# DocF/multispectral-object-detection

Measured on AMD Instinct MI355X. Metric: image-pairs/sec fwd, yolov5l+CFTx3 640×640 bs64, 1/2/4/8 GPU, higher is better.
Workload: dtype bf16; 1 GPU; cfg3 (yolov5l_fusion_transformerx3_FLIR_aligned) two-stream forward, 640x640, 64 pairs/GPU, BN folded, pre-NMS detections; pairs_per_gpu=64, image_size=640, parallelism=batch-shard x1, hip_graph=True, two_hip_streams=False, forwards_in_flight=3, streams_per_forward_in_flight=1, single_in_flight_streams=2

## Files before the change

include/cft_hip.h:

```cpp
#ifndef CFT_HIP_H
#define CFT_HIP_H

#ifdef __cplusplus
extern "C" {
#endif

#define CFT_ABI_VERSION 17

enum { CFT_BF16 = 0, CFT_F32 = 1, CFT_F16 = 2 };
enum { CFT_ACT_NONE = 0, CFT_ACT_SILU = 1, CFT_ACT_GELU = 2 };
enum {
  CFT_OK = 0,
  CFT_EINVAL = -1,
  CFT_ELAUNCH = -2,
  CFT_ENODEV = -3
};

int cft_abi_version(void);
int cft_device_check(void);
const char* cft_last_error(void);
int cft_clock_probe(void* out4_u64, int spin_us, int* wall_khz, void* stream);

int cft_conv2d(const void* x, const void* w, const float* bias, const void* res, void* y,
               int B, int H, int W, int cin, int ldx, int xoff,
               int n, int kpad, int ksize, int stride,
               int ldy, int yoff, int ldr, int roff,
               int act, int dtype, int out_dtype, int res_dtype, void* stream);

int cft_conv2d_chain(const void* x, const void* w1, const float* bias1, const void* w2, const float* bias2, void* y,
                     int B, int H, int W, int cin, int ldx, int xoff,
                     int n1, int kpad1, int ksize, int stride, int n2,
                     int ldy, int yoff, int act2, int dtype, void* stream);
int cft_conv2d_chain_ok(int B, int H, int W, int cin, int ldx, int n1, int kpad1, int ksize, int stride, int n2, int ldy, int dtype);

int cft_conv2d_chain_res(const void* x, const void* w1, const float* bias1, const void* res, void* y1,
                         const void* w2, const float* bias2, void* y2,
                         int B, int H, int W, int cin, int ldx, int xoff,
                         int n1, int kpad1, int ksize, int stride, int ldr, int roff, int ldy1, int yoff1,
                         int n2, int ldy2, int yoff2, int act2, int dtype, void* stream);

// ... 26 lines not shown
int cft_to_nhwc(const void* in, int in_dtype, long stride_b, long stride_c, long stride_h, long stride_w,
                void* out, int ldo, int ooff, int B, int C, int cpad, int H, int W, int dtype, void* stream);

int cft_letterbox_u8(const unsigned char* src, int src_h, int src_w, long src_row_stride,
                     unsigned char* dst, int dst_h, int dst_w, long dst_stride_y, long dst_stride_x, long dst_stride_c, int flip_channels,
                     int resized_h, int resized_w, int top, int left, int color0, int color1, int color2, void* stream);

enum { CFT_PAIR_COPY = 0, CFT_PAIR_LINEAR = 1, CFT_PAIR_AREA = 2 };
#define CFT_PAIR_DESC_BYTES 64
#define CFT_PAIR_MAX_REDUCTION 4
typedef struct {
  const unsigned char* src_rgb;
  const unsigned char* src_ir;
  long stride_rgb, stride_ir;
  int h0, w0;
  int h, w;
  int top, left;
  int mode, flip;
} cft_pair_desc_t;
int cft_pair_batch_u8(const void* desc_dev, const void* desc_host, int B, unsigned char* dst, int dst_h, int dst_w, int color, void* stream);

int cft_add(const void* a, int lda, int aoff, const void* b, int ldb, int boff,
            void* out, int ldo, int ooff, long M, int C, int dtype, void* stream);

int cft_gpt_tokenize(const void* rgb, int ld_rgb, int off_rgb, const void* ir, int ld_ir, int off_ir,
                     const float* pos_emb, float* tokens, int B, int H, int W, int C,
                     int dtype, void* stream);

int cft_layernorm(const float* x, const float* gamma, const float* beta, void* y,
                  long rows, int C, float eps, int out_dtype, void* stream);
int cft_layernorm_reduce(float* x, const float* parts, int nparts, const float* gamma, const float* beta, void* y,
                         long rows, int C, float eps, int out_dtype, void* stream);

int cft_attention(const void* qkv, void* out, int B, int heads, int dk, int dkp,
                  int dtype, float attn_pdrop, unsigned long long seed, void* stream);

int cft_gpt_upsample_add(const float* tokens, int s, const void* base, int ldb, int boff,
                         void* out, int ldo, int ooff, int B, int H, int W, int C,
                         int dtype, void* stream);

int cft_gpt_upsample_add2(const float* tokens, const void* base0, int ldb0, int boff0, const void* base1, int ldb1, int boff1,
                          void* out0, int ldo0, int ooff0, void* out1, int ldo1, int ooff1, void* sum, int lds, int soff,
                          int B, int H, int W, int C, int dtype, void* stream);

int cft_gpt_tokenize_grid(const void* rgb, int ld_rgb, int off_rgb, const void* ir, int ld_ir, int off_ir,
                          const float* pos_emb, float* tokens, int B, int H, int W, int C, int va, int ha,
                          int dtype, void* stream);

int cft_attention_tokens(const void* qkv, void* out, int B, int T, int heads, int dk, int dkp,
                         int dtype, float attn_pdrop, unsigned long long seed, void* stream);

int cft_gpt_upsample_add_grid(const float* tokens, int s, const void* base, int ldb, int boff,
                              void* out, int ldo, int ooff, int B, int H, int W, int C, int va, int ha,
                              int dtype, void* stream);

int cft_gpt_upsample_add2_grid(const float* tokens, const void* base0, int ldb0, int boff0, const void* base1, int ldb1, int boff1,
                               void* out0, int ldo0, int ooff0, void* out1, int ldo1, int ooff1, void* sum, int lds, int soff,
                               int B, int H, int W, int C, int va, int ha, int dtype, void* stream);

int cft_detect_decode(const float* logits, int ldl, float* raw, float* pred, const float* anchors,
                      int B, int ny, int nx, int na, int no, float stride,
                      long row0, long total_rows, void* stream);

long cft_batchnorm_train_workspace(long M, int C);
int cft_batchnorm_train(const float* x, int ldx, int xoff, long M, int C,
                        const float* gamma, const float* beta, float* running_mean, float* running_var,
// ... 48 lines not shown
```

multispectral-object-detection_amd/_lib.py:

```python
import ctypes
import os
import re
import subprocess

import torch

_HERE = os.path.dirname(os.path.abspath(__file__))
LIB_PATH = os.environ.get("CFT_HIP_LIB") or os.path.join(_HERE, "libcft_hip.so")
CSRC = os.path.join(_HERE, "csrc")
SOURCES = ("runtime.hip", "conv_gemm.hip", "conv_gemm_asm.hip", "focus_conv.hip", "bottleneck.hip", "pointwise.hip", "attention.hip", "attention_tokens.hip", "nms.hip", "train.hip", "metrics.hip", "confusion.hip", "loss.hip", "autoanchor.hip", "dataset.hip")

HEADER = os.path.join(_HERE, "..", "include", "cft_hip.h")
HEADERS = ("cft_common.h", "conv_common.h", "focus_common.h", "bneck_common.h", "metrics_common.h", "resize_common.h", "conv_gemm_asm.inc")

_SCALARS = {"int": ctypes.c_int, "long": ctypes.c_long, "float": ctypes.c_float, "unsigned long long": ctypes.c_ulonglong}
_RETURNS = {"int": ctypes.c_int, "long": ctypes.c_long, "const char*": ctypes.c_char_p}
_TYPE_WORDS = frozenset("void char short int long float double signed unsigned const".split())


def parse_header(text):
    text = re.sub(r"/\*.*?\*/|//[^\n]*", " ", text, flags=re.S)
    consts = {k: int(v) for k, v in re.findall(r"(?:#define\s+|\b)(CFT_\w+)\s*=?\s*(-?\d+)\b", text)}
    text = re.sub(r"^\s*#.*$", "", text, flags=re.M)
    sigs = {}
    for ret, name, args in re.findall(r"([\w\s*]+?)\b(cft_\w+)\s*\(([^()]*)\)\s*;", text):
        ret = re.sub(r"\s*\*", "*", " ".join(ret.split()))
        if ret not in _RETURNS:
            raise ValueError(f"{name}: unknown return type '{ret}'")
        argtypes = []
        for arg in ([] if args.strip() in ("", "void") else args.split(",")):
            *kind, pname = [w for w in arg.split() if w != "const"] or [""]
            if "*" in arg:
                argtypes.append(ctypes.c_void_p)
            elif " ".join(kind) in _SCALARS and pname not in _TYPE_WORDS:
                argtypes.append(_SCALARS[" ".join(kind)])
            else:
                raise ValueError(f"{name}: unknown parameter type in '{' '.join(arg.split())}' (scalars are named int / long / float / unsigned long long)")
        sigs[name] = (_RETURNS[ret], argtypes)
    return sigs, consts


with open(HEADER) as _fh:
    SIGNATURES, _consts = parse_header(_fh.read())
# ... 60 lines not shown
```

multispectral-object-detection_amd/csrc/cft_common.h:

```cpp
#pragma once
#include <hip/hip_runtime.h>
#include <stdint.h>
#include "../../include/cft_hip.h"

typedef __attribute__((ext_vector_type(8))) __bf16 bf16x8_t;
typedef __attribute__((ext_vector_type(4))) float f32x4_t;
typedef _Float16 f16_t;
typedef __attribute__((ext_vector_type(8))) _Float16 f16x8_t;
typedef __attribute__((ext_vector_type(2))) _Float16 f16x2_t;

typedef __attribute__((ext_vector_type(4))) uint32_t gran_t;

__device__ __forceinline__ float bf16_to_f32(uint16_t h) { return __uint_as_float(((uint32_t)h) << 16); }
__device__ __forceinline__ uint16_t f32_to_bf16(float f) {
  uint32_t u = __float_as_uint(f);
  if ((u & 0x7fffffffu) > 0x7f800000u) return (uint16_t)((u >> 16) | 0x40);
  u += 0x7fffu + ((u >> 16) & 1u);
  return (uint16_t)(u >> 16);
}
typedef __attribute__((ext_vector_type(2))) __bf16 bf16x2_t;
typedef __attribute__((ext_vector_type(2))) float f32x2_t;
__device__ __forceinline__ uint32_t pack_bf16x2(float lo, float hi) {
  return __builtin_bit_cast(uint32_t, __builtin_convertvector(f32x2_t{lo, hi}, bf16x2_t));
}
// ... 61 lines not shown
}
template <>
__device__ __forceinline__ f32x4_t mma_granule<f16_t>(const gran_t& a, const gran_t& b, f32x4_t c) {
  return __builtin_amdgcn_mfma_f32_16x16x32_f16(__builtin_bit_cast(f16x8_t, a), __builtin_bit_cast(f16x8_t, b), c, 0, 0, 0);
}
template <>
__device__ __forceinline__ f32x4_t mma_granule<float>(const gran_t& a, const gran_t& b, f32x4_t c) {
#pragma unroll
  for (int j = 0; j < 4; ++j)
    c = __builtin_amdgcn_mfma_f32_16x16x4f32(__uint_as_float(a[j]), __uint_as_float(b[j]), c, 0, 0, 0);
  return c;
}

__device__ __forceinline__ void lds_barrier() {
  asm volatile("s_waitcnt lgkmcnt(0)\n\ts_barrier" ::: "memory");
}

template <int ACT>
__device__ __forceinline__ float apply_act(float v) {
  if constexpr (ACT == CFT_ACT_SILU) return v * __builtin_amdgcn_rcpf(1.0f + __expf(-v));
  if constexpr (ACT == CFT_ACT_GELU) {
    const float z = fabsf(v) * 0.70710678118654752f;
    const float t = __builtin_amdgcn_rcpf(fmaf(0.3275911f, z, 1.0f));
    const float e = __builtin_amdgcn_exp2f(z * (z * -1.4426950408889634f));
    float q = fmaf(1.061405429f, t, -1.453152027f);
    q = fmaf(q, t, 1.421413741f);
    q = fmaf(q, t, -0.284496736f);
    q = fmaf(q, t, 0.254829592f);
    return fmaf(-0.5f * fabsf(v), q * t * e, fmaxf(v, 0.0f));
  }
  return v;
}

__device__ __forceinline__ uint32_t cft_hash32(unsigned long long seed, unsigned long long i) {
  unsigned long long z = seed + (i + 1ull) * 0x9E3779B97F4A7C15ull;
  z = (z ^ (z >> 30)) * 0xBF58476D1CE4E5B9ull;
  z = (z ^ (z >> 27)) * 0x94D049BB133111EBull;
  z = z ^ (z >> 31);
  return (uint32_t)(z >> 32);
}

void cft_set_error(const char* msg);
int cft_check_launch(const char* what);
static inline hipStream_t as_stream(void* s) { return (hipStream_t)s; }

template <auto Kernel>
static inline void cft_allow_lds(int bytes) {
  static bool done[64] = {};
  int dev = 0;
  if (hipGetDevice(&dev) != hipSuccess || dev < 0 || dev >= 64) {
    (void)hipFuncSetAttribute(reinterpret_cast<const void*>(Kernel), hipFuncAttributeMaxDynamicSharedMemorySize, bytes);
    return;
  }
  if (!done[dev]) {
    (void)hipFuncSetAttribute(reinterpret_cast<const void*>(Kernel), hipFuncAttributeMaxDynamicSharedMemorySize, bytes);
    done[dev] = true;
  }
}

static inline bool cft_is_dtype(int d) { return d == CFT_BF16 || d == CFT_F16 || d == CFT_F32; }
static inline int cft_elem_size(int d) { return d == CFT_F32 ? 4 : 2; }
static inline int cft_granule(int d) { return d == CFT_F32 ? 4 : 8; }

#define CFT_DISPATCH_DTYPE(dt_, T, ...)                              \
  do {                                                               \
    if ((dt_) == CFT_BF16) { using T = uint16_t; __VA_ARGS__; }      \
// ... 12 lines not shown
```

multispectral-object-detection_amd/csrc/pointwise.hip:

```cpp
#include "cft_common.h"
#include "resize_common.h"

static inline int grid_for(long work, int block) {
  long g = (work + block - 1) / block;
  const long cap = 256L * 16;
  return (int)(g < 1 ? 1 : (g > cap ? cap : g));
}

template <typename T>
__global__ void __launch_bounds__(256) focus_s2d_kernel(const float* __restrict__ in, unsigned char* __restrict__ out,
                                                        int B, int H, int W) {
  const int Ho = H >> 1, Wo = W >> 1;
  const long total = (long)B * Ho * Wo;
  for (long idx = (long)blockIdx.x * blockDim.x + threadIdx.x; idx < total; idx += (long)gridDim.x * blockDim.x) {
    const int x = (int)(idx % Wo);
    const long t = idx / Wo;
    const int y = (int)(t % Ho);
    const int b = (int)(t / Ho);
    float v[16];
#pragma unroll
    for (int c = 0; c < 3; ++c) {
      const float* base = in + (((long)b * 3 + c) * H + 2 * y) * W + 2 * x;
      const float2 top = *reinterpret_cast<const float2*>(base);
      const float2 bot = *reinterpret_cast<const float2*>(base + W);
// ... 328 lines not shown
        Elem<T>::unpack(*reinterpret_cast<const gran_t*>(src + (((long)b * H + y) * W + x) * ldb + offb + cg * 16L), f);
#pragma unroll
        for (int e = 0; e < GE; ++e) acc[e] += f[e];
      }
    float* o = tokens + ((long)b * 128 + cell) * C + cg * GE;
    const float* pe = pos_emb + (long)cell * C + cg * GE;
#pragma unroll
    for (int e = 0; e < GE; ++e) o[e] = acc[e] * inv + pe[e];
  }
}

extern "C" int cft_gpt_tokenize(const void* rgb, int ld_rgb, int off_rgb, const void* ir, int ld_ir, int off_ir,
                                const float* pos_emb, float* tokens, int B, int H, int W, int C,
                                int dtype, void* stream) {
  CFT_REQUIRE(rgb && ir && pos_emb && tokens, "cft_gpt_tokenize: null pointer");
  CFT_REQUIRE(cft_is_dtype(dtype), "cft_gpt_tokenize: bad dtype");
  const int ge = cft_granule(dtype), es = cft_elem_size(dtype);
  CFT_REQUIRE(C % ge == 0 && ld_rgb % ge == 0 && off_rgb % ge == 0 && ld_ir % ge == 0 && off_ir % ge == 0, "cft_gpt_tokenize: not granule aligned");
  CFT_REQUIRE(B > 0 && H >= 1 && W >= 1, "cft_gpt_tokenize: bad shape");
  int threads = C / ge;
  threads = threads < 64 ? 64 : (threads > 256 ? 256 : ((threads + 63) / 64) * 64);
  CFT_DISPATCH_DTYPE(dtype, T, hipLaunchKernelGGL(gpt_tokenize_kernel<T>, dim3(B * 128), dim3(threads), 0, as_stream(stream), (const unsigned char*)rgb, (long)ld_rgb * es, (long)off_rgb * es,
                                                   (const unsigned char*)ir, (long)ld_ir * es, (long)off_ir * es, pos_emb, tokens, H, W, C));
  return cft_check_launch("gpt_tokenize_kernel");
}

template <int MAXV>
__global__ void __launch_bounds__(256) layernorm_kernel(const float* __restrict__ x, const float* __restrict__ gamma,
                                                        const float* __restrict__ beta, unsigned char* __restrict__ y,
                                                        long rows, int C, float eps, int out_dtype) {
  const int lane = threadIdx.x & 63;
  const long row = (long)blockIdx.x * 4 + (threadIdx.x >> 6);
  if (row >= rows) return;
  const int nv = C >> 2;
  const float4* xr = reinterpret_cast<const float4*>(x + row * C);
  float4 v[MAXV];
  float s = 0.f;
#pragma unroll
  for (int k = 0; k < MAXV; ++k) {
    const int idx = lane + k * 64;
    v[k] = idx < nv ? xr[idx] : make_float4(0.f, 0.f, 0.f, 0.f);
    s += v[k].x + v[k].y + v[k].z + v[k].w;
  }
#pragma unroll
  for (int o = 32; o > 0; o >>= 1) s += __shfl_xor(s, o);
  const float mean = s / (float)C;
  float q = 0.f;
#pragma unroll
  for (int k = 0; k < MAXV; ++k) {
    const int idx = lane + k * 64;
    if (idx < nv) {
      const float a = v[k].x - mean, b = v[k].y - mean, c = v[k].z - mean, d = v[k].w - mean;
      q += a * a + b * b + c * c + d * d;
    }
  }
#pragma unroll
  for (int o = 32; o > 0; o >>= 1) q += __shfl_xor(q, o);
  const float rstd = rsqrtf(q / (float)C + eps);
#pragma unroll
  for (int k = 0; k < MAXV; ++k) {
    const int idx = lane + k * 64;
    if (idx < nv) {
      const float4 gm = reinterpret_cast<const float4*>(gamma)[idx];
      const float4 bt = reinterpret_cast<const float4*>(beta)[idx];
      float o[4] = {(v[k].x - mean) * rstd * gm.x + bt.x, (v[k].y - mean) * rstd * gm.y + bt.y,
                    (v[k].z - mean) * rstd * gm.z + bt.z, (v[k].w - mean) * rstd * gm.w + bt.w};
      if (out_dtype == CFT_F32) {
        *reinterpret_cast<float4*>(y + (row * C + idx * 4L) * 4) = *reinterpret_cast<float4*>(o);
      } else {
        uint2 pk;
        if (out_dtype == CFT_BF16) { pk.x = pack_bf16x2(o[0], o[1]); pk.y = pack_bf16x2(o[2], o[3]); }
        else { pk.x = pack_f16x2(o[0], o[1]); pk.y = pack_f16x2(o[2], o[3]); }
        *reinterpret_cast<uint2*>(y + (row * C + idx * 4L) * 2) = pk;
      }
    }
  }
}

template <int MAXV>
__global__ void __launch_bounds__(256) layernorm_reduce_kernel(float* __restrict__ x, const float* __restrict__ parts, int nparts, long part_stride,
                                                               const float* __restrict__ gamma, const float* __restrict__ beta,
                                                               unsigned char* __restrict__ y, long rows, int C, float eps, int out_dtype) {
  const int lane = threadIdx.x & 63;
  const long row = (long)blockIdx.x * 4 + (threadIdx.x >> 6);
  if (row >= rows) return;
  const int nv = C >> 2;
  float4* xr = reinterpret_cast<float4*>(x + row * C);
  float4 v[MAXV];
  float s = 0.f;
#pragma unroll
  for (int k = 0; k < MAXV; ++k) {
    const int idx = lane + k * 64;
    v[k] = make_float4(0.f, 0.f, 0.f, 0.f);
    if (idx < nv) {
      float4 a = xr[idx];
      for (int sp = 0; sp < nparts; ++sp) {
        const float4 q = reinterpret_cast<const float4*>(parts + sp * part_stride + row * C)[idx];
        a.x += q.x; a.y += q.y; a.z += q.z; a.w += q.w;
      }
      xr[idx] = a;
      v[k] = a;
    }
    s += v[k].x + v[k].y + v[k].z + v[k].w;
  }
#pragma unroll
  for (int o = 32; o > 0; o >>= 1) s += __shfl_xor(s, o);
  const float mean = s / (float)C;
  float q = 0.f;
#pragma unroll
// ... 454 lines not shown
```

multispectral-object-detection_amd/models/common.py:

```python
import math

import torch
import torch.nn as nn

from .. import ops
from ..ops import ACT_GELU, ACT_NONE, ACT_SILU

BN_EPS = 1e-3


def autopad(k, p=None):
    if p is None:
        p = k // 2 if isinstance(k, int) else [x // 2 for x in k]
    return p


class _Pending:

    def materialize(self):
        raise NotImplementedError


class PendingBilinear(_Pending):

# ... 368 lines not shown
        self.que_proj = nn.Linear(d_model, h * self.d_k)
        self.key_proj = nn.Linear(d_model, h * self.d_k)
        self.val_proj = nn.Linear(d_model, h * self.d_v)
        self.out_proj = nn.Linear(h * self.d_v, d_model)
        self.attn_drop = nn.Dropout(attn_pdrop)
        self.resid_drop = nn.Dropout(resid_pdrop)
        for m in (self.que_proj, self.key_proj, self.val_proj, self.out_proj):
            nn.init.normal_(m.weight, std=0.001)
            nn.init.constant_(m.bias, 0)

    @staticmethod
    def padded_head(dk, dtype):
        step = 16 if dtype == torch.float32 else 32
        return ((dk + step - 1) // step) * step

    def _pack(self, dtype, device):
        h, dk, d = self.h, self.d_k, self.d_model
        dkp = self.padded_head(dk, dtype)
        ws, bs = [], []
        for lin in (self.que_proj, self.key_proj, self.val_proj):
            w = torch.zeros((h, dkp, d), dtype=torch.float32, device=device)
            b = torch.zeros((h, dkp), dtype=torch.float32, device=device)
            w[:, :dk] = lin.weight.detach().float().to(device).view(h, dk, d)
            b[:, :dk] = lin.bias.detach().float().to(device).view(h, dk)
            ws.append(w.view(h * dkp, d))
            bs.append(b.view(h * dkp))
        qkv = ops.pack_conv(torch.cat(ws, 0), torch.cat(bs, 0), dtype, device=device, n_true=3 * h * dk)
        wo = torch.zeros((d, h, dkp), dtype=torch.float32, device=device)
        wo[:, :, :dk] = self.out_proj.weight.detach().float().to(device).view(d, h, dk)
        out = ops.pack_conv(wo.view(d, h * dkp), self.out_proj.bias, dtype, device=device)
        out.flops_per_row = 2.0 * d * h * dk
        return qkv, out, dkp

    def forward(self, x, attention_mask=None, attention_weights=None, residual=None, splitk=False, ntok=128):
        if attention_mask is not None or attention_weights is not None:
            raise NotImplementedError("attention_mask / attention_weights are unused by GPT (reference :497-500)")
        qkv_w, out_w, dkp = self._packed(x.dtype, x.device)
        B = x.shape[0] // ntok
        qkv = ops.linear(x, qkv_w)
        att = ops.attention(qkv, B, self.h, self.d_k, dkp, pdrop=self.attn_drop.p if self.training else 0.0, T=ntok)
        if self.training and self.resid_drop.p > 0 and residual is not None:
            proj = ops.linear(att, out_w, out_dtype=torch.float32)
            ops.dropout_(proj, self.resid_drop.p)
            return ops.add_rows_(residual, proj)
        if splitk and residual is not None and not self.training:
            s_ = ops.splitk_choice(att.shape[0], out_w, att.dtype)
            if s_ > 1:
                return ops.linear_splitk(att, out_w, s_)
        out = ops.linear(att, out_w, residual=residual, out=residual,
                         out_dtype=torch.float32 if residual is not None else None)
        return None if splitk else out


class myTransformerBlock(_Packed):

    def __init__(self, d_model, d_k, d_v, h, block_exp, attn_pdrop, resid_pdrop):
        super().__init__()
        self.ln_input = nn.LayerNorm(d_model)
        self.ln_output = nn.LayerNorm(d_model)
        self.sa = SelfAttention(d_model, d_k, d_v, h, attn_pdrop, resid_pdrop)
        self.mlp = nn.Sequential(
            nn.Linear(d_model, block_exp * d_model),
            nn.GELU(),
            nn.Linear(block_exp * d_model, d_model),
            nn.Dropout(resid_pdrop),
        )

    def _pack(self, dtype, device):
        fc1 = ops.pack_conv(self.mlp[0].weight, self.mlp[0].bias, dtype, device=device)
        fc2 = ops.pack_conv(self.mlp[2].weight, self.mlp[2].bias, dtype, device=device)
        ln = [_f32(t, device) for t in (self.ln_input.weight, self.ln_input.bias, self.ln_output.weight, self.ln_output.bias)]
        return fc1, fc2, ln

    splitk = True

    def forward(self, x, compute_dtype=torch.bfloat16, pending=None, ntok=128):
        fc1, fc2, ln = self._packed(compute_dtype, x.device)
        split = self.splitk and not self.training and x.is_cuda

        def norm(parts, g, b, eps):
            if parts is not None:
                return ops.layernorm_reduce(x, parts, g, b, compute_dtype, eps)
            return ops.layernorm(x, g, b, compute_dtype, eps)
        y = norm(pending, ln[0], ln[1], self.ln_input.eps)
        parts = None
        if split:
            parts = self.sa(y, residual=x, splitk=True, ntok=ntok)
        else:
            self.sa(y, residual=x, ntok=ntok)
        y = norm(parts, ln[2], ln[3], self.ln_output.eps)
        hid = ops.linear(y, fc1, act=ACT_GELU)
        pd = self.mlp[3].p if (self.training and len(self.mlp) > 3) else 0.0
        if pd > 0:
            z = ops.linear(hid, fc2, out_dtype=torch.float32)
            ops.dropout_(z, pd)
            ops.add_rows_(x, z)
            return None
        if split:
            s_ = ops.splitk_choice(hid.shape[0], fc2, hid.dtype)
            if s_ > 1:
                return ops.linear_splitk(hid, fc2, s_)
        ops.linear(hid, fc2, residual=x, out=x, out_dtype=torch.float32)
        return None


class GPT(_Packed):

    def __init__(self, d_model, h=8, block_exp=4, n_layer=8, vert_anchors=8, horz_anchors=8,
                 embd_pdrop=0.1, attn_pdrop=0.1, resid_pdrop=0.1):
        super().__init__()
        self.n_embd = d_model
        self.vert_anchors = vert_anchors
        self.horz_anchors = horz_anchors
        d_k = d_model
        d_v = d_model
        self.pos_emb = nn.Parameter(torch.zeros(1, 2 * vert_anchors * horz_anchors, self.n_embd))
        self.trans_blocks = nn.Sequential(*[myTransformerBlock(d_model, d_k, d_v, h, block_exp, attn_pdrop, resid_pdrop)
# ... 14 lines not shown
            module.weight.data.fill_(1.0)

    def _pack(self, dtype, device):
        return _f32(self.pos_emb, device), _f32(self.ln_f.weight, device), _f32(self.ln_f.bias, device)

    def check_supported(self, C=None):
        grid = (int(self.vert_anchors), int(self.horz_anchors))
        if grid != (self.vert_anchors, self.horz_anchors):
            raise NotImplementedError(f"anchor grid {self.vert_anchors}x{self.horz_anchors}: vert_anchors / horz_anchors must be integers")
        ops._grid(grid)
        blk = self.trans_blocks[0] if len(self.trans_blocks) else None
        if blk is not None and blk.sa.d_k > 256:
            raise NotImplementedError(f"GPT head width d_model / h = {blk.sa.d_k}: the attention kernels take head widths <= 256")
        C = self.n_embd if C is None else C
        if grid != ops.ANCHOR_GRID and C > 2048:
            raise NotImplementedError(f"GPT d_model = {C} on a {grid[0]}x{grid[1]} anchor grid: the kernels take d_model <= 2048")
        return grid

    def forward(self, x):
        grid = self.check_supported()
        T = 2 * grid[0] * grid[1]
        rgb, ir = resolve(x[0]), resolve(x[1])
        assert rgb.shape[0] == ir.shape[0]
        if rgb.shape != ir.shape or rgb.dtype != ir.dtype:
            raise ValueError("GPT: the two streams must have the same shape and dtype")
        B, C, H, W = rgb.shape
        dtype = rgb.dtype
        pos_emb, lnf_w, lnf_b = self._packed(dtype, rgb.device)
        tok = ops.gpt_tokenize(rgb, ir, pos_emb, grid=grid)
        if self.training:
            ops.dropout_(tok, self.drop.p)
        t2 = tok.view(B * T, C)
        pending = None
        for blk in self.trans_blocks:
            pending = blk(t2, dtype, pending, ntok=T)
        if pending is not None:
            tok_f = ops.layernorm_reduce(t2, pending, lnf_w, lnf_b, torch.float32, self.ln_f.eps).view(B, T, C)
        else:
            tok_f = ops.layernorm(t2, lnf_w, lnf_b, torch.float32, self.ln_f.eps).view(B, T, C)
        tok_f.anchor_grid = grid
        return PendingBilinear(tok_f, 0, H, W, dtype, grid), PendingBilinear(tok_f, 1, H, W, dtype, grid)


def _outside(name, where):
    def __init__(self, *a, **k):
        raise NotImplementedError(f"{name} (reference {where}) is outside the two-stream CFT hot path; "
                                  "no fusion yaml uses it (SURVEY.md section 2)")
    return type(name, (nn.Module,), {"__init__": __init__, "__doc__": f"Placeholder for the reference's {name} ({where})."})


def DWConv(c1, c2, k=1, s=1, act=True):
    raise NotImplementedError("DWConv (grouped convolution) is outside the two-stream CFT hot path")


TransformerLayer = _outside("TransformerLayer", "models/common.py:53-67")
TransformerBlock = _outside("TransformerBlock", "models/common.py:70-96")
BottleneckCSP = _outside("BottleneckCSP", "models/common.py:112-128")
C3TR = _outside("C3TR", "models/common.py:146-151")
Contract = _outside("Contract", "models/common.py:183-194")
Expand = _outside("Expand", "models/common.py:197-208")


class NMS(nn.Module):
    conf = 0.25
    iou = 0.45
    classes = None

    def forward(self, x):
        from ..utils.general import non_max_suppression
# ... 69 lines not shown
```

multispectral-object-detection_amd/ops.py:

```python
from dataclasses import dataclass
from typing import Optional

import torch

from . import _lib
from ._lib import ACT_GELU, ACT_NONE, ACT_SILU, CFT_BF16, CFT_F16, CFT_F32


COMPUTE_DTYPES = (torch.bfloat16, torch.float16, torch.float32)


def _dt(dtype):
    if dtype == torch.bfloat16:
        return CFT_BF16
    if dtype == torch.float16:
        return CFT_F16
    if dtype == torch.float32:
        return CFT_F32
    raise TypeError(f"compute dtype must be torch.bfloat16, torch.float16 or torch.float32, got {dtype}")


def _stream():
    return torch.cuda.current_stream().cuda_stream


def _require_cuda(t, what):
    if not t.is_cuda:
        raise RuntimeError(f"{what}: tensor is on {t.device}; this package runs on MI355X only "
                           "(no CPU fallback - use oracle/ for a CPU reference)")


def granule(dtype):
# ... 301 lines not shown
        best = s
        if t256 * s >= 128:
            break
    return best


def linear_splitk(x, pk, splits):
    _require_cuda(x, "linear_splitk")
    rows, K = x.shape
    if K != pk.cin or x.stride(1) != 1:
        raise ValueError(f"linear_splitk: input [{rows},{K}] does not match packed weight (cin {pk.cin})")
    parts = torch.empty((splits, rows, pk.n), dtype=torch.float32, device=x.device)
    lib = _lib.load()
    abytes = rows * K * x.element_size() + splits * rows * pk.n_valid * 4 + pk.w.numel() * x.element_size()
    st = _timed(f"linear_k{pk.k}s{pk.s}_n{pk.n}_K{pk.kpad}", rows * pk.flops_per_row, abytes,
                lambda: lib.cft_linear_splitk(x.data_ptr(), pk.w.data_ptr(), _bias_ptr(pk), parts.data_ptr(),
                                              rows, pk.cin, x.stride(0), pk.n, pk.kpad, splits, _dt(x.dtype), _stream()))
    _lib.check(st, "cft_linear_splitk")
    return parts


def layernorm_reduce(x, parts, gamma, beta, out_dtype, eps=1e-5):
    _require_cuda(x, "layernorm_reduce")
    rows, C = x.shape
    if parts.dtype != torch.float32 or tuple(parts.shape[1:]) != (rows, C) or not parts.is_contiguous() or not x.is_contiguous() or x.dtype != torch.float32:
        raise ValueError(f"layernorm_reduce: x {tuple(x.shape)} {x.dtype} / parts {tuple(parts.shape)} {parts.dtype} must be contiguous fp32 with matching rows")
    out = torch.empty((rows, C), dtype=out_dtype, device=x.device)
    lib = _lib.load()
    st = _timed("cft_layernorm", 0.0, rows * C * (8.0 + 4.0 * parts.shape[0] + out.element_size()),
                lambda: lib.cft_layernorm_reduce(x.data_ptr(), parts.data_ptr(), parts.shape[0], gamma.data_ptr(), beta.data_ptr(), out.data_ptr(),
                                                 rows, C, eps, _dt(out_dtype), _stream()))
    _lib.check(st, "cft_layernorm_reduce")
    return out


def focus_s2d(img, dtype):
    _require_cuda(img, "focus_s2d")
    if img.dtype == torch.uint8:
        B, C, H, W = img.shape
        if C != 3 or img.stride(3) != 1:
            raise ValueError("focus_s2d: uint8 input must be [B,3,H,W] with contiguous rows")
        out = new_nhwc(B, H // 2, W // 2, 16, dtype, img.device)
        st = _lib.load().cft_focus_s2d_u8(img.data_ptr(), img.stride(0), img.stride(1), img.stride(2), out.data_ptr(),
                                          B, H, W, 1.0 / 255.0, _dt(dtype), _stream())
        _lib.check(st, "cft_focus_s2d_u8")
        return out
    B, C, H, W = img.shape
    if C != 3:
        raise ValueError(f"focus_s2d: expected 3 input channels, got {C}")
    if img.dtype != torch.float32 or not img.is_contiguous():
        if img.dtype not in COMPUTE_DTYPES:
            raise TypeError(f"focus_s2d: unsupported image dtype {img.dtype}")
        if W % 4:
            raise ValueError("focus_s2d: image width must be a multiple of 4")
        flat = torch.empty((B, 3, H, W), dtype=torch.float32, device=img.device)
        lib, es = _lib.load(), img.element_size()
        sb, sc, sh, sw = img.stride()
        if sb == 3 * sc:
            calls = [(img.data_ptr(), flat.data_ptr(), (sc, sw, sh, 0), B * 3, H)]
        elif sc == H * sh:
            calls = [(img.data_ptr(), flat.data_ptr(), (sb, sw, sh, 0), B, 3 * H)]
        else:
            calls = [(img.data_ptr() + b * sb * es, flat.data_ptr() + b * 3 * H * W * 4, (sc, sw, sh, 0), 3, H) for b in range(B)]
        for src, dst, (s0, s1, s2, s3), nb, nh in calls:
            _lib.check(lib.cft_to_nhwc(src, _dt(img.dtype), s0, s1, s2, s3, dst, W, 0, nb, W, W, nh, 1, CFT_F32, _stream()),
                       "cft_to_nhwc(image)")
# ... 290 lines not shown
```

Baseline: 3647 image-pairs/sec.

## Fuse transformer block tail (out-proj, residual, LN, MLP, next LN) into one kernel

Adds a fused HIP kernel that runs, per 32-row tile, the attention output projection with bias and residual, then the post-attention layernorm, the fc1+GELU and fc2 MLP with a second residual, and the next block's (or final) input layernorm. The intermediate hidden activations stay in LDS and are never written to global memory. It is enabled by default for d=256 with at least 8192 token rows in inference, and replaces several separate linear, split-k reduce and layernorm launches per GPT block. The trade-off is a large-LDS, 512-thread kernel with heavy register use whose occupancy and MFMA efficiency may fall below the tuned standalone GEMMs. The layernorm row code is also moved into a shared helper.

```diff
diff --git a/include/cft_hip.h b/include/cft_hip.h
--- a/include/cft_hip.h
+++ b/include/cft_hip.h
@@ -5,7 +5,7 @@
 extern "C" {
 #endif
 
-#define CFT_ABI_VERSION 17
+#define CFT_ABI_VERSION 18
 
 enum { CFT_BF16 = 0, CFT_F32 = 1, CFT_F16 = 2 };
 enum { CFT_ACT_NONE = 0, CFT_ACT_SILU = 1, CFT_ACT_GELU = 2 };
@@ -98,6 +98,13 @@
 int cft_layernorm_reduce(float* x, const float* parts, int nparts, const float* gamma, const float* beta, void* y,
                          long rows, int C, float eps, int out_dtype, void* stream);
 
+int cft_block_tail(const void* att, int ld_att, float* x, const void* wo, const float* bo, const float* ln_g, const float* ln_b,
+                   const void* w1, const float* b1, const void* w2, const float* b2,
+                   const float* next_g, const float* next_b, void* y_next, int y_next_dtype,
+                   long rows, int d, int hidden, int k_o, float eps, float next_eps, int dtype, void* stream);
+int cft_block_tail_ok(long rows, int d, int hidden, int k_o, int ld_att, int dtype);
+int cft_block_tail_rows(int d);
+
 int cft_attention(const void* qkv, void* out, int B, int heads, int dk, int dkp,
                   int dtype, float attn_pdrop, unsigned long long seed, void* stream);
 
diff --git a/multispectral-object-detection_amd/_lib.py b/multispectral-object-detection_amd/_lib.py
--- a/multispectral-object-detection_amd/_lib.py
+++ b/multispectral-object-detection_amd/_lib.py
@@ -8,7 +8,7 @@
 _HERE = os.path.dirname(os.path.abspath(__file__))
 LIB_PATH = os.environ.get("CFT_HIP_LIB") or os.path.join(_HERE, "libcft_hip.so")
 CSRC = os.path.join(_HERE, "csrc")
-SOURCES = ("runtime.hip", "conv_gemm.hip", "conv_gemm_asm.hip", "focus_conv.hip", "bottleneck.hip", "pointwise.hip", "attention.hip", "attention_tokens.hip", "nms.hip", "train.hip", "metrics.hip", "confusion.hip", "loss.hip", "autoanchor.hip", "dataset.hip")
+SOURCES = ("runtime.hip", "conv_gemm.hip", "conv_gemm_asm.hip", "focus_conv.hip", "bottleneck.hip", "pointwise.hip", "attention.hip", "attention_tokens.hip", "cft_tail.hip", "nms.hip", "train.hip", "metrics.hip", "confusion.hip", "loss.hip", "autoanchor.hip", "dataset.hip")
 
 HEADER = os.path.join(_HERE, "..", "include", "cft_hip.h")
 HEADERS = ("cft_common.h", "conv_common.h", "focus_common.h", "bneck_common.h", "metrics_common.h", "resize_common.h", "conv_gemm_asm.inc")
diff --git a/multispectral-object-detection_amd/csrc/cft_common.h b/multispectral-object-detection_amd/csrc/cft_common.h
--- a/multispectral-object-detection_amd/csrc/cft_common.h
+++ b/multispectral-object-detection_amd/csrc/cft_common.h
@@ -117,6 +117,57 @@
   return v;
 }
 
+template <int MAXV, typename Store>
+__device__ __forceinline__ void layernorm_row(const float4* xr, const float* __restrict__ gamma, const float* __restrict__ beta,
+                                              int nv, int C, float eps, int lane, Store&& store) {
+#pragma clang fp contract(off)
+  float4 v[MAXV];
+  float s = 0.f;
+#pragma unroll
+  for (int k = 0; k < MAXV; ++k) {
+    const int idx = lane + k * 64;
+    v[k] = idx < nv ? xr[idx] : make_float4(0.f, 0.f, 0.f, 0.f);
+    s += v[k].x + v[k].y + v[k].z + v[k].w;
+  }
+#pragma unroll
+  for (int o = 32; o > 0; o >>= 1) s += __shfl_xor(s, o);
+  const float mean = s / (float)C;
+  float q = 0.f;
+#pragma unroll
+  for (int k = 0; k < MAXV; ++k) {
+    const int idx = lane + k * 64;
+    if (idx < nv) {
+      const float a = v[k].x - mean, b = v[k].y - mean, c = v[k].z - mean, d = v[k].w - mean;
+      q += a * a + b * b + c * c + d * d;
+    }
+  }
+#pragma unroll
+  for (int o = 32; o > 0; o >>= 1) q += __shfl_xor(q, o);
+  const float rstd = rsqrtf(q / (float)C + eps);
+#pragma unroll
+  for (int k = 0; k < MAXV; ++k) {
+    const int idx = lane + k * 64;
+    if (idx < nv) {
+      const float4 gm = reinterpret_cast<const float4*>(gamma)[idx];
+      const float4 bt = reinterpret_cast<const float4*>(beta)[idx];
+      float o[4] = {fmaf((v[k].x - mean) * rstd, gm.x, bt.x), fmaf((v[k].y - mean) * rstd, gm.y, bt.y),
+                    fmaf((v[k].z - mean) * rstd, gm.z, bt.z), fmaf((v[k].w - mean) * rstd, gm.w, bt.w)};
+      store(idx, o);
+    }
+  }
+}
+
+__device__ __forceinline__ void layernorm_store(unsigned char* __restrict__ y, long row, int C, int idx, float (&o)[4], int out_dtype) {
+  if (out_dtype == CFT_F32) {
+    *reinterpret_cast<float4*>(y + (row * C + idx * 4L) * 4) = *reinterpret_cast<float4*>(o);
+  } else {
+    uint2 pk;
+    if (out_dtype == CFT_BF16) { pk.x = pack_bf16x2(o[0], o[1]); pk.y = pack_bf16x2(o[2], o[3]); }
+    else { pk.x = pack_f16x2(o[0], o[1]); pk.y = pack_f16x2(o[2], o[3]); }
+    *reinterpret_cast<uint2*>(y + (row * C + idx * 4L) * 2) = pk;
+  }
+}
+
 __device__ __forceinline__ uint32_t cft_hash32(unsigned long long seed, unsigned long long i) {
   unsigned long long z = seed + (i + 1ull) * 0x9E3779B97F4A7C15ull;
   z = (z ^ (z >> 30)) * 0xBF58476D1CE4E5B9ull;
diff --git a/multispectral-object-detection_amd/csrc/cft_tail.hip b/multispectral-object-detection_amd/csrc/cft_tail.hip
--- /dev/null
+++ b/multispectral-object-detection_amd/csrc/cft_tail.hip
@@ -0,0 +1,252 @@
+#include "cft_common.h"
+
+struct TailParams {
+  const unsigned char* att;
+  long ld_att;
+  float* x;
+  const unsigned char *wo, *w1, *w2;
+  const float *bo, *b1, *b2, *ln_g, *ln_b, *next_g, *next_b;
+  unsigned char* y_next;
+  int y_next_dtype;
+  long rows;
+  float eps, next_eps;
+};
+
+template <typename T, int MT, int NTX, int FP>
+__device__ __forceinline__ void tail_mma(f32x4_t (&acc)[MT][NTX], const gran_t (&b)[FP], const unsigned char* a_lane, int astride, int f0,
+                                         const int (&sw)[4]) {
+  static_assert(FP % NTX == 0, "a piece holds whole k-steps");
+  gran_t af[MT];
+#pragma unroll
+  for (int fi = 0; fi < FP; ++fi) {
+    const int kk = (f0 + fi) / NTX, j = (f0 + fi) % NTX;
+    if (j == 0) {
+#pragma unroll
+      for (int i = 0; i < MT; ++i)
+        af[i] = *reinterpret_cast<const gran_t*>(a_lane + i * 16 * astride + sw[kk & 3] + (kk >> 2) * 256);
+    }
+#pragma unroll
+    for (int i = 0; i < MT; ++i) acc[i][j] = mma_granule<T>(af[i], b[fi], acc[i][j]);
+  }
+}
+
+template <typename T, int D, int R, int HC, int FP>
+__global__ void __launch_bounds__(512) block_tail_kernel(const TailParams p) {
+  constexpr int HID = 4 * D, NCH = HID / HC;
+  constexpr int WN = D / 8, NT = WN / 16, MT = R / 16;
+  constexpr int WN1 = HC / 8, NT1 = WN1 / 16;
+  constexpr int P0 = (D / 32) * NT / FP, P1 = (D / 32) * NT1 / FP, P2 = (HC / 32) * NT / FP, PPC = P1 + P2;
+  constexpr int UNR = NCH <= 4 ? NCH : 2;
+  constexpr int AHEAD = NT <= 2 ? 3 : 2;
+  constexpr int XS = D * 4, HS = HC * 2, HB = R * HS;
+  static_assert(NT >= 1 && NT1 >= 1 && MT >= 1 && PPC % 4 == 0 && P0 >= 1 && P1 >= 1 && P2 >= 1 && HC % 128 == 0, "tile shape");
+  static_assert(((D / 32) * NT) % FP == 0 && ((D / 32) * NT1) % FP == 0 && ((HC / 32) * NT) % FP == 0, "pieces");
+  typedef typename Half16<T>::type TH;
+  extern __shared__ __attribute__((aligned(16))) unsigned char smem[];
+  unsigned char* sX = smem;
+  unsigned char* sH = smem + R * XS;
+
+  const int tid = threadIdx.x, lane = tid & 63;
+  const int wave = __builtin_amdgcn_readfirstlane(tid >> 6);
+  const int lrow = lane & 15, lgrp = lane >> 4;
+  const long m0 = (long)blockIdx.x * R;
+
+  const unsigned char* wo_l = p.wo + ((long)(wave * WN + lrow) * D + lgrp * 8) * 2;
+  const unsigned char* w1_l = p.w1 + ((long)(wave * WN1 + lrow) * D + lgrp * 8) * 2;
+  const unsigned char* w2_l = p.w2 + ((long)(wave * WN + lrow) * HID + lgrp * 8) * 2;
+  auto load_mlp = [&](gran_t (&dst)[FP], int c, int r) {
+#pragma unroll
+    for (int fi = 0; fi < FP; ++fi) {
+      if (r < P1) {
+        const int f = r * FP + fi, kk = f / NT1, j = f % NT1;
+        dst[fi] = *reinterpret_cast<const gran_t*>(w1_l + (long)c * (HC * D * 2) + j * (16 * D * 2) + kk * 64);
+      } else {
+        const int f = (r - P1) * FP + fi, kk = f / NT, j = f % NT;
+        dst[fi] = *reinterpret_cast<const gran_t*>(w2_l + (long)c * (HC * 2) + j * (16 * HID * 2) + kk * 64);
+      }
+    }
+  };
+  auto load_piece = [&](gran_t (&dst)[FP], int g) {
+    if (g < P0) {
+#pragma unroll
+      for (int fi = 0; fi < FP; ++fi) {
+        const int f = g * FP + fi, kk = f / NT, j = f % NT;
+        dst[fi] = *reinterpret_cast<const gran_t*>(wo_l + j * (16 * D * 2) + kk * 64);
+      }
+    } else {
+      load_mlp(dst, (g - P0) / PPC, (g - P0) % PPC);
+    }
+  };
+
+  constexpr int GPR = D / 8;
+  constexpr int A_PER = R * GPR / 512;
+  static_assert((R * GPR) % 512 == 0, "att staging");
+  gran_t ra[A_PER];
+#pragma unroll
+  for (int i = 0; i < A_PER; ++i) {
+    const int idx = tid + i * 512, row = idx / GPR, g = idx % GPR;
+    ra[i] = gran_t{0u, 0u, 0u, 0u};
+    if (m0 + row < p.rows) ra[i] = *reinterpret_cast<const gran_t*>(p.att + ((m0 + row) * p.ld_att + g * 8) * 2);
+  }
+  gran_t ring[4][FP];
+#pragma unroll
+  for (int g = 0; g < AHEAD; ++g) load_piece(ring[g], g);
+  f32x4_t xres[MT][NT];
+  float bo_v[NT], b2_v[NT];
+#pragma unroll
+  for (int j = 0; j < NT; ++j) {
+    const int col = wave * WN + j * 16 + lrow;
+    bo_v[j] = p.bo[col];
+    b2_v[j] = p.b2[col];
+#pragma unroll
+    for (int i = 0; i < MT; ++i)
+#pragma unroll
+      for (int e = 0; e < 4; ++e) {
+        const long m = m0 + i * 16 + lgrp * 4 + e;
+        xres[i][j][e] = m < p.rows ? p.x[m * D + col] : 0.0f;
+      }
+  }
+#pragma unroll
+  for (int i = 0; i < A_PER; ++i) {
+    const int idx = tid + i * 512, row = idx / GPR, g = idx % GPR;
+    *reinterpret_cast<gran_t*>(sX + row * XS + ((g ^ (row & 15)) << 4)) = ra[i];
+  }
+  __syncthreads();
+
+  const unsigned char* ax_lane = sX + lrow * XS;
+  int sw[4];
+#pragma unroll
+  for (int q = 0; q < 4; ++q) sw[q] = ((q * 4 + lgrp) ^ lrow) << 4;
+  f32x4_t acc2[MT][NT];
+#pragma unroll
+  for (int i = 0; i < MT; ++i)
+#pragma unroll
+    for (int j = 0; j < NT; ++j) acc2[i][j] = f32x4_t{0.f, 0.f, 0.f, 0.f};
+#pragma unroll
+  for (int g = 0; g < P0; ++g) {
+    load_piece(ring[(g + AHEAD) & 3], g + AHEAD);
+    tail_mma<T, MT, NT, FP>(acc2, ring[g & 3], ax_lane, XS, g * FP, sw);
+  }
+  auto residual_rows = [&](f32x4_t (&acc)[MT][NT], const float (&bias_v)[NT]) {
+    __syncthreads();
+#pragma unroll
+    for (int i = 0; i < MT; ++i)
+#pragma unroll
+      for (int j = 0; j < NT; ++j)
+#pragma unroll
+        for (int e = 0; e < 4; ++e) {
+          const float v = acc[i][j][e] + bias_v[j];
+          xres[i][j][e] = v + xres[i][j][e];
+          *reinterpret_cast<float*>(sX + (i * 16 + lgrp * 4 + e) * XS + (wave * WN + j * 16 + lrow) * 4) = xres[i][j][e];
+          acc[i][j][e] = 0.f;
+        }
+    __syncthreads();
+  };
+  residual_rows(acc2, bo_v);
+  for (int row = wave; row < R; row += 8) {
+    unsigned char* xr = sX + row * XS;
+    layernorm_row<2>(reinterpret_cast<const float4*>(xr), p.ln_g, p.ln_b, D / 4, D, p.eps, lane, [&](int idx, float (&o)[4]) {
+      uint2 pk;
+      pk.x = Elem<TH>::pack2(o[0], o[1]);
+      pk.y = Elem<TH>::pack2(o[2], o[3]);
+      *reinterpret_cast<uint2*>(xr + (((idx >> 1) ^ (row & 15)) << 4) + (idx & 1) * 8) = pk;
+    });
+  }
+  __syncthreads();
+
+#pragma unroll UNR
+  for (int c = 0; c < NCH; ++c) {
+    float b1_v[NT1];
+#pragma unroll
+    for (int j = 0; j < NT1; ++j) b1_v[j] = p.b1[c * HC + wave * WN1 + j * 16 + lrow];
+    f32x4_t acc1[MT][NT1];
+#pragma unroll
+    for (int i = 0; i < MT; ++i)
+#pragma unroll
+      for (int j = 0; j < NT1; ++j) acc1[i][j] = f32x4_t{0.f, 0.f, 0.f, 0.f};
+    unsigned char* hbuf = sH + (c & 1) * HB;
+#pragma unroll
+    for (int r = 0; r < PPC; ++r) {
+      constexpr int S0 = P0 & 3;
+      if (r + AHEAD < PPC) load_mlp(ring[(S0 + r + AHEAD) & 3], c, r + AHEAD);
+      else if (c + 1 < NCH) load_mlp(ring[(S0 + r + AHEAD) & 3], c + 1, r + AHEAD - PPC);
+      if (r < P1) {
+        tail_mma<T, MT, NT1, FP>(acc1, ring[(S0 + r) & 3], ax_lane, XS, r * FP, sw);
+      } else {
+        tail_mma<T, MT, NT, FP>(acc2, ring[(S0 + r) & 3], hbuf + lrow * HS, HS, (r - P1) * FP, sw);
+      }
+      if (r == P1 - 1) {
+#pragma unroll
+        for (int i = 0; i < MT; ++i)
+#pragma unroll
+          for (int j = 0; j < NT1; ++j)
+#pragma unroll
+            for (int e = 0; e < 4; ++e) {
+              float v = apply_act<CFT_ACT_GELU>(acc1[i][j][e] + b1_v[j]);
+              asm volatile("" : "+v"(v));
+              const int row = i * 16 + lgrp * 4 + e, col = wave * WN1 + j * 16 + lrow;
+              *reinterpret_cast<uint16_t*>(hbuf + row * HS + (((col >> 3) ^ (row & 15)) << 4) + (col & 7) * 2) = (uint16_t)Elem<TH>::pack2(v, 0.0f);
+            }
+        __syncthreads();
+      }
+    }
+  }
+  residual_rows(acc2, b2_v);
+  constexpr int VPR = D / 4;
+  for (int idx = tid; idx < R * VPR; idx += 512) {
+    const int row = idx / VPR, v4 = idx % VPR;
+    if (m0 + row < p.rows)
+      reinterpret_cast<float4*>(p.x + (m0 + row) * D)[v4] = reinterpret_cast<const float4*>(sX + row * XS)[v4];
+  }
+  if (p.y_next != nullptr) {
+    for (int row = wave; row < R; row += 8) {
+      const long m = m0 + row;
+      if (m >= p.rows) break;
+      layernorm_row<2>(reinterpret_cast<const float4*>(sX + row * XS), p.next_g, p.next_b, D / 4, D, p.next_eps, lane,
+                       [&](int idx, float (&o)[4]) { layernorm_store(p.y_next, m, D, idx, o, p.y_next_dtype); });
+    }
+  }
+}
+
+extern "C" int cft_block_tail_rows(int d) { return (d == 256 || d == 512) ? 32 : 0; }
+
+extern "C" int cft_block_tail_ok(long rows, int d, int hidden, int k_o, int ld_att, int dtype) {
+  if (dtype != CFT_BF16 && dtype != CFT_F16) return 0;
+  if (cft_block_tail_rows(d) == 0 || hidden != 4 * d || k_o != d) return 0;
+  if (ld_att < d || ld_att % 8 != 0) return 0;
+  if (rows <= 0 || (rows + 31) / 32 >= (1L << 31)) return 0;
+  return 1;
+}
+
+template <typename T, int D, int R, int HC, int FP>
+static int launch_tail(const TailParams& p, hipStream_t stream) {
+  constexpr int LDS = R * D * 4 + 2 * R * HC * 2;
+  static_assert(LDS <= 160 * 1024, "LDS");
+  cft_allow_lds<block_tail_kernel<T, D, R, HC, FP>>(LDS);
+  hipLaunchKernelGGL((block_tail_kernel<T, D, R, HC, FP>), dim3((unsigned)((p.rows + R - 1) / R)), dim3(512), LDS, stream, p);
+  return cft_check_launch("block_tail_kernel");
+}
+
+extern "C" int cft_block_tail(const void* att, int ld_att, float* x, const void* wo, const float* bo, const float* ln_g, const float* ln_b,
+                              const void* w1, const float* b1, const void* w2, const float* b2,
+                              const float* next_g, const float* next_b, void* y_next, int y_next_dtype,
+                              long rows, int d, int hidden, int k_o, float eps, float next_eps, int dtype, void* stream) {
+  CFT_REQUIRE(cft_block_tail_ok(rows, d, hidden, k_o, ld_att, dtype), "cft_block_tail: shape not eligible (bf16 / fp16, d in {256, 512}, hidden == 4 d, k_o == d, ld_att >= d)");
+  CFT_REQUIRE(att && x && wo && bo && ln_g && ln_b && w1 && b1 && w2 && b2, "cft_block_tail: null pointer");
+  CFT_REQUIRE(y_next == nullptr || (next_g && next_b && cft_is_dtype(y_next_dtype)), "cft_block_tail: y_next needs next_g / next_b and a dtype");
+  CFT_REQUIRE(((uintptr_t)att | (uintptr_t)x | (uintptr_t)wo | (uintptr_t)w1 | (uintptr_t)w2 | (uintptr_t)y_next | (uintptr_t)ln_g | (uintptr_t)ln_b |
+               (uintptr_t)next_g | (uintptr_t)next_b) % 16 == 0, "cft_block_tail: pointers must be 16-byte aligned");
+  TailParams p;
+  p.att = (const unsigned char*)att; p.ld_att = ld_att; p.x = x;
+  p.wo = (const unsigned char*)wo; p.w1 = (const unsigned char*)w1; p.w2 = (const unsigned char*)w2;
+  p.bo = bo; p.b1 = b1; p.b2 = b2; p.ln_g = ln_g; p.ln_b = ln_b; p.next_g = next_g; p.next_b = next_b;
+  p.y_next = (unsigned char*)y_next; p.y_next_dtype = y_next_dtype;
+  p.rows = rows; p.eps = eps; p.next_eps = next_eps;
+  hipStream_t s = as_stream(stream);
+  if (d == 256) {
+    if (dtype == CFT_BF16) return launch_tail<uint16_t, 256, 32, 256, 8>(p, s);
+    return launch_tail<f16_t, 256, 32, 256, 8>(p, s);
+  }
+  if (dtype == CFT_BF16) return launch_tail<uint16_t, 512, 32, 128, 4>(p, s);
+  return launch_tail<f16_t, 512, 32, 128, 4>(p, s);
+}
diff --git a/multispectral-object-detection_amd/csrc/pointwise.hip b/multispectral-object-detection_amd/csrc/pointwise.hip
--- a/multispectral-object-detection_amd/csrc/pointwise.hip
+++ b/multispectral-object-detection_amd/csrc/pointwise.hip
@@ -384,49 +384,8 @@
   const int lane = threadIdx.x & 63;
   const long row = (long)blockIdx.x * 4 + (threadIdx.x >> 6);
   if (row >= rows) return;
-  const int nv = C >> 2;
   const float4* xr = reinterpret_cast<const float4*>(x + row * C);
-  float4 v[MAXV];
-  float s = 0.f;
-#pragma unroll
-  for (int k = 0; k < MAXV; ++k) {
-    const int idx = lane + k * 64;
-    v[k] = idx < nv ? xr[idx] : make_float4(0.f, 0.f, 0.f, 0.f);
-    s += v[k].x + v[k].y + v[k].z + v[k].w;
-  }
-#pragma unroll
-  for (int o = 32; o > 0; o >>= 1) s += __shfl_xor(s, o);
-  const float mean = s / (float)C;
-  float q = 0.f;
-#pragma unroll
-  for (int k = 0; k < MAXV; ++k) {
-    const int idx = lane + k * 64;
-    if (idx < nv) {
-      const float a = v[k].x - mean, b = v[k].y - mean, c = v[k].z - mean, d = v[k].w - mean;
-      q += a * a + b * b + c * c + d * d;
-    }
-  }
-#pragma unroll
-  for (int o = 32; o > 0; o >>= 1) q += __shfl_xor(q, o);
-  const float rstd = rsqrtf(q / (float)C + eps);
-#pragma unroll
-  for (int k = 0; k < MAXV; ++k) {
-    const int idx = lane + k * 64;
-    if (idx < nv) {
-      const float4 gm = reinterpret_cast<const float4*>(gamma)[idx];
-      const float4 bt = reinterpret_cast<const float4*>(beta)[idx];
-      float o[4] = {(v[k].x - mean) * rstd * gm.x + bt.x, (v[k].y - mean) * rstd * gm.y + bt.y,
-                    (v[k].z - mean) * rstd * gm.z + bt.z, (v[k].w - mean) * rstd * gm.w + bt.w};
-      if (out_dtype == CFT_F32) {
-        *reinterpret_cast<float4*>(y + (row * C + idx * 4L) * 4) = *reinterpret_cast<float4*>(o);
-      } else {
-        uint2 pk;
-        if (out_dtype == CFT_BF16) { pk.x = pack_bf16x2(o[0], o[1]); pk.y = pack_bf16x2(o[2], o[3]); }
-        else { pk.x = pack_f16x2(o[0], o[1]); pk.y = pack_f16x2(o[2], o[3]); }
-        *reinterpret_cast<uint2*>(y + (row * C + idx * 4L) * 2) = pk;
-      }
-    }
-  }
+  layernorm_row<MAXV>(xr, gamma, beta, C >> 2, C, eps, lane, [&](int idx, float (&o)[4]) { layernorm_store(y, row, C, idx, o, out_dtype); });
 }
 
 template <int MAXV>
diff --git a/multispectral-object-detection_amd/models/common.py b/multispectral-object-detection_amd/models/common.py
--- a/multispectral-object-detection_amd/models/common.py
+++ b/multispectral-object-detection_amd/models/common.py
@@ -424,13 +424,16 @@
         out.flops_per_row = 2.0 * d * h * dk
         return qkv, out, dkp
 
+    def attend(self, x, ntok=128):
+        qkv_w, out_w, dkp = self._packed(x.dtype, x.device)
+        qkv = ops.linear(x, qkv_w)
+        att = ops.attention(qkv, x.shape[0] // ntok, self.h, self.d_k, dkp, pdrop=self.attn_drop.p if self.training else 0.0, T=ntok)
+        return att, out_w
+
     def forward(self, x, attention_mask=None, attention_weights=None, residual=None, splitk=False, ntok=128):
         if attention_mask is not None or attention_weights is not None:
             raise NotImplementedError("attention_mask / attention_weights are unused by GPT (reference :497-500)")
-        qkv_w, out_w, dkp = self._packed(x.dtype, x.device)
-        B = x.shape[0] // ntok
-        qkv = ops.linear(x, qkv_w)
-        att = ops.attention(qkv, B, self.h, self.d_k, dkp, pdrop=self.attn_drop.p if self.training else 0.0, T=ntok)
+        att, out_w = self.attend(x, ntok)
         if self.training and self.resid_drop.p > 0 and residual is not None:
             proj = ops.linear(att, out_w, out_dtype=torch.float32)
             ops.dropout_(proj, self.resid_drop.p)
@@ -466,7 +469,34 @@
 
     splitk = True
 
+    def tail_ok(self, x, compute_dtype):
+        if not (ops.CFT_TAIL and not self.training and x.is_cuda and x.shape[0] >= ops.CFT_TAIL_MIN_ROWS and x.shape[1] in ops.CFT_TAIL_WIDTHS):
+            return False
+        fc1, fc2, _ = self._packed(compute_dtype, x.device)
+        out_w = self.sa._packed(compute_dtype, x.device)[1]
+        if not ops.block_tail_ok(x.shape[0], x.shape[1], out_w, fc1, fc2, compute_dtype):
+            return False
+        return not self.splitk or (ops.splitk_choice(x.shape[0], out_w, compute_dtype) == 1 and ops.splitk_choice(x.shape[0], fc2, compute_dtype) == 1)
+
     def forward(self, x, compute_dtype=torch.bfloat16, pending=None, ntok=128):
+        return self.run(x, compute_dtype, pending, ntok)[0]
+
+    def run(self, x, compute_dtype=torch.bfloat16, pending=None, ntok=128, y_in=None, next_ln=None):
+        if self.tail_ok(x, compute_dtype):
+            fc1, fc2, ln = self._packed(compute_dtype, x.device)
+            if y_in is None:
+                y_in = (ops.layernorm(x, ln[0], ln[1], compute_dtype, self.ln_input.eps) if pending is None else
+                        ops.layernorm_reduce(x, pending, ln[0], ln[1], compute_dtype, self.ln_input.eps))
+            att, out_w = self.sa.attend(y_in, ntok)
+            g, b, eps, dt = next_ln if next_ln is not None else (None, None, 1e-5, None)
+            return None, ops.block_tail(att, x, out_w, ln[2], ln[3], fc1, fc2, g, b, dt, self.ln_output.eps, eps)
+        return self._run_unfused(x, compute_dtype, pending, ntok, y_in), None
+
+    def ln_input_args(self, compute_dtype, device):
+        ln = self._packed(compute_dtype, device)[2]
+        return ln[0], ln[1], self.ln_input.eps, compute_dtype
+
+    def _run_unfused(self, x, compute_dtype, pending, ntok, y_in=None):
         fc1, fc2, ln = self._packed(compute_dtype, x.device)
         split = self.splitk and not self.training and x.is_cuda
 
@@ -474,7 +504,7 @@
             if parts is not None:
                 return ops.layernorm_reduce(x, parts, g, b, compute_dtype, eps)
             return ops.layernorm(x, g, b, compute_dtype, eps)
-        y = norm(pending, ln[0], ln[1], self.ln_input.eps)
+        y = y_in if y_in is not None else norm(pending, ln[0], ln[1], self.ln_input.eps)
         parts = None
         if split:
             parts = self.sa(y, residual=x, splitk=True, ntok=ntok)
@@ -555,9 +585,18 @@
             ops.dropout_(tok, self.drop.p)
         t2 = tok.view(B * T, C)
         pending = None
-        for blk in self.trans_blocks:
-            pending = blk(t2, dtype, pending, ntok=T)
-        if pending is not None:
+        y = None
+        blocks = list(self.trans_blocks)
+        fused = [blk.tail_ok(t2, dtype) for blk in blocks]
+        for j, blk in enumerate(blocks):
+            nxt = None
+            if fused[j]:
+                nxt = ((lnf_w, lnf_b, self.ln_f.eps, torch.float32) if j + 1 == len(blocks) else
+                       blocks[j + 1].ln_input_args(dtype, rgb.device) if fused[j + 1] else None)
+            pending, y = blk.run(t2, dtype, pending, ntok=T, y_in=y, next_ln=nxt)
+        if y is not None:
+            tok_f = y.view(B, T, C)
+        elif pending is not None:
             tok_f = ops.layernorm_reduce(t2, pending, lnf_w, lnf_b, torch.float32, self.ln_f.eps).view(B, T, C)
         else:
             tok_f = ops.layernorm(t2, lnf_w, lnf_b, torch.float32, self.ln_f.eps).view(B, T, C)
diff --git a/multispectral-object-detection_amd/ops.py b/multispectral-object-detection_amd/ops.py
--- a/multispectral-object-detection_amd/ops.py
+++ b/multispectral-object-detection_amd/ops.py
@@ -1,3 +1,4 @@
+import os
 from dataclasses import dataclass
 from typing import Optional
 
@@ -365,6 +366,53 @@
                                                  rows, C, eps, _dt(out_dtype), _stream()))
     _lib.check(st, "cft_layernorm_reduce")
     return out
+
+
+CFT_TAIL = os.environ.get("MSOD_CFT_TAIL", "1") != "0"
+CFT_TAIL_MIN_ROWS = 8192
+CFT_TAIL_WIDTHS = (256,)
+
+
+def _tail_args(out_w, fc1, fc2):
+    return all(pk.k == 1 and pk.kpad == pk.cin and pk.bias is not None and pk.n == pk.n_valid for pk in (out_w, fc1, fc2))
+
+
+def block_tail_ok(rows, d, out_w, fc1, fc2, dtype, ld_att=None):
+    if dtype not in (torch.bfloat16, torch.float16) or not _tail_args(out_w, fc1, fc2):
+        return False
+    if not (out_w.n == d == fc1.cin == fc2.n and fc2.cin == fc1.n) or out_w.w.dtype != dtype or fc1.w.dtype != dtype or fc2.w.dtype != dtype:
+        return False
+    return bool(_lib.load().cft_block_tail_ok(rows, d, fc1.n, out_w.cin, out_w.cin if ld_att is None else ld_att, _dt(dtype)))
+
+
+def block_tail_rows(d):
+    return _lib.load().cft_block_tail_rows(d)
+
+
+def block_tail(att, x, out_w, ln_g, ln_b, fc1, fc2, next_g=None, next_b=None, next_dtype=None, eps=1e-5, next_eps=1e-5):
+    _require_cuda(att, "block_tail")
+    rows, d = x.shape
+    if att.shape[0] != rows or att.stride(1) != 1 or x.dtype != torch.float32 or not x.is_contiguous():
+        raise ValueError(f"block_tail: att {tuple(att.shape)} / x {tuple(x.shape)} {x.dtype}: x must be contiguous fp32 with att's rows")
+    if not _tail_args(out_w, fc1, fc2) or att.shape[1] != out_w.cin or not (out_w.n == d == fc1.cin == fc2.n and fc2.cin == fc1.n):
+        raise ValueError("block_tail: packed weights must be un-padded pointwise layers with a bias, att as wide as out_proj's input")
+    y_next = None
+    if next_g is not None:
+        y_next = torch.empty((rows, d), dtype=next_dtype or att.dtype, device=x.device)
+    lib = _lib.load()
+    es = att.element_size()
+    flops = rows * (out_w.flops_per_row + fc1.flops_per_row + fc2.flops_per_row)
+    abytes = (rows * out_w.cin * es + 2 * rows * d * 4 + (0 if y_next is None else rows * d * y_next.element_size())
+              + (out_w.w.numel() + fc1.w.numel() + fc2.w.numel()) * es)
+    st = _timed(f"linear_tail_d{d}", flops, abytes,
+                lambda: lib.cft_block_tail(att.data_ptr(), att.stride(0), x.data_ptr(), out_w.w.data_ptr(), out_w.bias.data_ptr(),
+                                           ln_g.data_ptr(), ln_b.data_ptr(), fc1.w.data_ptr(), fc1.bias.data_ptr(), fc2.w.data_ptr(),
+                                           fc2.bias.data_ptr(), None if next_g is None else next_g.data_ptr(),
+                                           None if next_b is None else next_b.data_ptr(), None if y_next is None else y_next.data_ptr(),
+                                           _dt(y_next.dtype) if y_next is not None else CFT_F32, rows, d, fc1.n, out_w.cin, eps, next_eps,
+                                           _dt(att.dtype), _stream()))
+    _lib.check(st, "cft_block_tail")
+    return y_next
 
 
 def focus_s2d(img, dtype):
```

Result: no change. 3644 image-pairs/sec (-0.1%).
